# Dhia-naouali/dinov3-jax

Hardware: NVIDIA H100
Metric: global_crops_per_sec (higher is better)
Workload: dtype bf16

## Files before the change

dinov3-jax_b200/csrc/gemm_tc.cu:

```cuda
#include <cstdlib>
#include <cstring>
#include "ptx.cuh"
#include "d3_internal.h"

namespace d3 {

constexpr int BM = 128;
constexpr int BK = 64;
constexpr int GEMM_THREADS = 384;

constexpr int EPI_RUNTIME = -1;
constexpr int EPI_FLAGS = EP_BIAS | EP_GELU | EP_STORE_PRE | EP_MUL_DGELU | EP_GAMMA | EP_RESID | EP_OUT_F32 | EP_ACCUM |
                          EP_SLABS | EP_GELU_ERF;

template <int EF>
constexpr bool kStaged = EF != EPI_RUNTIME && (EF & (EP_SLABS | EP_ACCUM)) == 0;

template <int EF>
__device__ __forceinline__ bool epi_has(const GemmEpilogue& ep, int f) {
  return EF == EPI_RUNTIME ? (ep.flags & f) != 0 : (EF & f) != 0;
}

__device__ __forceinline__ float gelu_grad_epi(float u) {
  const float u2 = __fmul_rn(u, u);
  const float t = tanh_approx(__fmul_rn(u, fmaf(0.0356774081363001f, u2, 0.7978845608028654f)));
  const float dz = fmaf(0.1070322244089003f, u2, 0.7978845608028654f);
  return fmaf(__fmul_rn(__fmul_rn(0.5f, u), fmaf(-t, t, 1.0f)), dz, __fmul_rn(0.5f, __fadd_rn(1.0f, t)));
}

__device__ __forceinline__ float gelu_erf_epi(float u) {
  return __fmul_rn(__fmul_rn(0.5f, u), __fadd_rn(1.0f, erff(__fmul_rn(u, 0.70710678118654752f))));
}

template <int EF>
__device__ __forceinline__ float epi_value(const GemmEpilogue& ep, float acc, float bias, float u, float gamma,
                                           float resid, float old, float& pre) {
  float v = __fmul_rn(acc, ep.alpha);
  if (epi_has<EF>(ep, EP_BIAS)) v = __fadd_rn(v, bias);
  pre = v;
  if (epi_has<EF>(ep, EP_GELU)) v = gelu_tanh_fast(v);
  if (epi_has<EF>(ep, EP_GELU_ERF)) v = gelu_erf_epi(v);
  if (epi_has<EF>(ep, EP_MUL_DGELU)) v = __fmul_rn(v, gelu_grad_epi(u));
  if (epi_has<EF>(ep, EP_GAMMA)) v = __fmul_rn(v, gamma);
  if (epi_has<EF>(ep, EP_RESID)) v = __fadd_rn(v, resid);
  if (epi_has<EF>(ep, EP_ACCUM)) v = __fadd_rn(v, old);
  return v;
}

__device__ __forceinline__ float2 ld_pair(const float* p, bool vec, bool two) {
  if (vec) return *reinterpret_cast<const float2*>(p);
  return make_float2(p[0], two ? p[1] : 0.f);
}
__device__ __forceinline__ float2 ld_pair(const __nv_bfloat16* p, bool vec, bool two) {
  if (vec) return unpack_bf16(*reinterpret_cast<const uint32_t*>(p));
  return make_float2(__bfloat162float(p[0]), two ? __bfloat162float(p[1]) : 0.f);
}
__device__ __forceinline__ void st_pair(float* p, float a, float b, bool vec, bool two) {
  if (vec) {
    *reinterpret_cast<float2*>(p) = make_float2(a, b);
  } else {
    p[0] = a;
    if (two) p[1] = b;
  }
}
__device__ __forceinline__ void st_pair(__nv_bfloat16* p, float a, float b, bool vec, bool two) {
  if (vec) {
    *reinterpret_cast<uint32_t*>(p) = pack_bf16(a, b);
  } else {
    p[0] = __float2bfloat16(a);
    if (two) p[1] = __float2bfloat16(b);
  }
}

template <int BN>
__device__ __forceinline__ void epilogue_tile_runtime(const GemmEpilogue& ep, float (&acc)[2][BN / 2], int m0, int n0,
                                                      int M, int N, size_t slab_row0, int r_in, int c_in) {
  float* const out_f = reinterpret_cast<float*>(ep.out);
  __nv_bfloat16* const out_h = reinterpret_cast<__nv_bfloat16*>(ep.out);
  const bool aligned = (ep.flags & EP_SLOW) == 0;
#pragma unroll
  for (int mh = 0; mh < 2; ++mh)
#pragma unroll
    for (int h = 0; h < 2; ++h) {
      const size_t row = (size_t)(m0 + mh * 64 + r_in + 8 * h);
      if (row >= (size_t)M) continue;
      const size_t orow = slab_row0 + row;
#pragma unroll
      for (int i = 0; i < BN / 8; ++i) {
        const int n = n0 + 8 * i + c_in;
        if (n >= N) break;
        const bool two = n + 1 < N, vec = aligned && two;
        float2 b{}, u{}, g{}, x{}, o{};
        if (epi_has<EPI_RUNTIME>(ep, EP_BIAS)) b = ld_pair(ep.bias + n, vec, two);
        if (epi_has<EPI_RUNTIME>(ep, EP_MUL_DGELU)) u = ld_pair(ep.aux_in + row * ep.ld_aux + n, vec, two);
        if (epi_has<EPI_RUNTIME>(ep, EP_GAMMA)) g = ld_pair(ep.gamma + n, vec, two);
        if (epi_has<EPI_RUNTIME>(ep, EP_RESID)) x = ld_pair(ep.resid + row * ep.ld_resid + n, vec, two);
        if (epi_has<EPI_RUNTIME>(ep, EP_ACCUM)) o = ld_pair(out_f + orow * ep.ld_out + n, vec, two);
        float p0, p1;
        const float v0 = epi_value<EPI_RUNTIME>(ep, acc[mh][4 * i + 2 * h], b.x, u.x, g.x, x.x, o.x, p0);
        const float v1 = epi_value<EPI_RUNTIME>(ep, acc[mh][4 * i + 2 * h + 1], b.y, u.y, g.y, x.y, o.y, p1);
        if (epi_has<EPI_RUNTIME>(ep, EP_SCATTER)) {
          const unsigned long long g_idx = (unsigned long long)ep.sc_off + orow * ep.ld_out + n;
          const unsigned long long shard = (unsigned long long)ep.sc_shard;
          const unsigned r = (unsigned)(g_idx / shard);
          float* const dst = ep.sc_peer[r] + (g_idx - r * shard);
          if (!two) atomicAdd(dst, v0);
          else atomicAdd(reinterpret_cast<float2*>(dst), make_float2(v0, v1));
          continue;
        }
        if (epi_has<EPI_RUNTIME>(ep, EP_STORE_PRE)) st_pair(ep.aux_out + row * ep.ld_aux + n, p0, p1, vec, two);
        if (epi_has<EPI_RUNTIME>(ep, EP_OUT_F32)) st_pair(out_f + orow * ep.ld_out + n, v0, v1, vec, two);
        else st_pair(out_h + orow * ep.ld_out + n, v0, v1, vec, two);
      }
    }
}

constexpr int STG_BOX = 64 * 128;
constexpr int STG_BYTES = 3 * STG_BOX;
__device__ __forceinline__ uint32_t sw128(int r, int byte) {
  return r * 128 + ((((byte >> 4) ^ r) & 7) << 4) + (byte & 15);
}

template <int MH, int BN, int EF>
__device__ __forceinline__ void epilogue_tile(const GemmEpilogue& ep, const CUtensorMap* tm_out,
                                              const CUtensorMap* tm_pre, float (&acc)[MH][BN / 2], const float* s_bias,
                                              const float* s_gamma, uint8_t* stg, int& seq, int bar, int t, int m0,
                                              int n0, int M, int N, size_t slab_row0, int r_in, int c_in) {
  constexpr bool STAGED = kStaged<EF>;
  constexpr bool F32 = (EF & EP_OUT_F32) != 0;
  constexpr int OUT_BOXES = F32 ? 2 : 1;
  constexpr int CHUNK = (OUT_BOXES + ((EF & EP_STORE_PRE) ? 1 : 0)) * STG_BOX;
  constexpr int NBUF = STG_BYTES / CHUNK;
  static_assert(NBUF >= 1, "a chunk must fit the staging area");
  float* const out_f = reinterpret_cast<float*>(ep.out);
  __nv_bfloat16* const out_h = reinterpret_cast<__nv_bfloat16*>(ep.out);
#pragma unroll
  for (int mh = 0; mh < MH; ++mh)
#pragma unroll
    for (int cb = 0; cb < BN / 64; ++cb) {
      const int row0 = m0 + mh * 64, col0 = n0 + cb * 64;
      if (row0 >= M || col0 >= N) continue;
      float2 xr[2][8], xo[2][8];
      uint32_t xu[2][8];
#pragma unroll
      for (int h = 0; h < 2; ++h) {
        const size_t row = (size_t)row0 + r_in + 8 * h;
#pragma unroll
        for (int i = 0; i < 8; ++i) {
          const int n = col0 + 8 * i + c_in;
          if (row < (size_t)M && n < N) {
            if (epi_has<EF>(ep, EP_RESID))
              xr[h][i] = *reinterpret_cast<const float2*>(ep.resid + row * ep.ld_resid + n);
            if (epi_has<EF>(ep, EP_MUL_DGELU))
              xu[h][i] = *reinterpret_cast<const uint32_t*>(ep.aux_in + row * ep.ld_aux + n);
            if (epi_has<EF>(ep, EP_ACCUM))
              xo[h][i] = *reinterpret_cast<const float2*>(out_f + (slab_row0 + row) * ep.ld_out + n);
          }
        }
      }
      uint8_t* const buf = stg + (seq % NBUF) * CHUNK;
      if constexpr (STAGED) {
        if (t == 0) tma_store_wait_read<NBUF - 1>();
        named_bar_sync(bar, 128);
      }
#pragma unroll
      for (int h = 0; h < 2; ++h) {
        const int r = r_in + 8 * h;
        const size_t row = (size_t)row0 + r;
#pragma unroll
        for (int i = 0; i < 8; ++i) {
          const int cl = cb * 64 + 8 * i + c_in;
          const int n = n0 + cl;
          const float2 b = epi_has<EF>(ep, EP_BIAS) ? *reinterpret_cast<const float2*>(s_bias + cl) : float2{};
          const float2 g = epi_has<EF>(ep, EP_GAMMA) ? *reinterpret_cast<const float2*>(s_gamma + cl) : float2{};
          const float2 u = epi_has<EF>(ep, EP_MUL_DGELU) ? unpack_bf16(xu[h][i]) : float2{};
          float p0, p1;
          const float v0 = epi_value<EF>(ep, acc[mh][4 * (cl >> 3) + 2 * h], b.x, u.x, g.x, xr[h][i].x, xo[h][i].x, p0);
          const float v1 = epi_value<EF>(ep, acc[mh][4 * (cl >> 3) + 2 * h + 1], b.y, u.y, g.y, xr[h][i].y, xo[h][i].y,
                                         p1);
          if constexpr (STAGED) {
            if (epi_has<EF>(ep, EP_STORE_PRE))
              *reinterpret_cast<uint32_t*>(buf + OUT_BOXES * STG_BOX + sw128(r, 16 * i + 2 * c_in)) = pack_bf16(p0, p1);
            if constexpr (F32) {
              *reinterpret_cast<float2*>(buf + (i >> 2) * STG_BOX + sw128(r, 32 * (i & 3) + 4 * c_in)) =
                  make_float2(v0, v1);
            } else {
              *reinterpret_cast<uint32_t*>(buf + sw128(r, 16 * i + 2 * c_in)) = pack_bf16(v0, v1);
            }
          } else if (row < (size_t)M && n < N) {
            if (epi_has<EF>(ep, EP_STORE_PRE)) st_pair(ep.aux_out + row * ep.ld_aux + n, p0, p1, true, true);
            if constexpr (F32) st_pair(out_f + (slab_row0 + row) * ep.ld_out + n, v0, v1, true, true);
            else st_pair(out_h + (slab_row0 + row) * ep.ld_out + n, v0, v1, true, true);
          }
        }
      }
      if constexpr (STAGED) {
        fence_proxy_async_smem();
        named_bar_sync(bar, 128);
        if (t == 0) {
          tma_store_2d(tm_out, buf, col0, row0);
          if (F32 && col0 + 32 < N) tma_store_2d(tm_out, buf + STG_BOX, col0 + 32, row0);
          if constexpr ((EF & EP_STORE_PRE) != 0) tma_store_2d(tm_pre, buf + OUT_BOXES * STG_BOX, col0, row0);
          tma_store_commit();
        }
        ++seq;
      }
    }
}

template <int BN, bool STAGED>
struct Cfg {
  static constexpr bool WIDE = BN == 256;
  static constexpr int STAGES = (BN == 256 ? 4 : BN == 128 ? 6 : 8) - (STAGED ? 1 : 0);
  static constexpr int A_BYTES = BM * BK * 2;
  static constexpr int B_BYTES = BN * BK * 2;
  static constexpr int STAGE_BYTES = A_BYTES + B_BYTES;
  static constexpr int BAR_BYTES = 256;
  static constexpr int VEC_BYTES = (WIDE ? 1 : 2) * 2 * BN * 4;
  static constexpr int VEC_END = STAGES * STAGE_BYTES + BAR_BYTES + VEC_BYTES;
  static constexpr int STG_OFF = (VEC_END + 1023) / 1024 * 1024;
  static constexpr int SMEM_BYTES = (STAGED ? STG_OFF + 2 * STG_BYTES : VEC_END) + 1024;
  static_assert(SMEM_BYTES <= 227 * 1024, "over the opt-in shared-memory limit");
};

struct WorkRange { int m0, n0, kb0, kb1, sp; };
template <int BN>
__device__ __forceinline__ WorkRange work_item(int w, int rank, int num_n, int num_tiles, int num_k, int splits) {
  const int tile = w % num_tiles, sp = w / num_tiles;
  const int per = (num_k + splits - 1) / splits;
  WorkRange r;
  if constexpr (BN == 256) {
    r.n0 = (tile % num_n) * BN;
    r.m0 = (2 * (tile / num_n) + rank) * BM;
  } else {
    r.n0 = (2 * (tile % num_n) + rank) * BN;
    r.m0 = (tile / num_n) * BM;
  }
  r.kb0 = sp * per;
  r.kb1 = min(num_k, r.kb0 + per);
  r.sp = sp;
  return r;
}

template <int MH, int BN, int A_MN, int B_MN>
__device__ __forceinline__ void mma_kblock(float (&acc)[MH][BN / 2], uint32_t sa, uint32_t sb, bool first) {
  const uint64_t bd = B_MN ? gmma_desc_sw128(sb, 8192, 1024) : gmma_desc_sw128(sb, 16, 1024);
  constexpr uint64_t a_adv = A_MN ? (2048 >> 4) : (32 >> 4);
  constexpr uint64_t b_adv = B_MN ? (2048 >> 4) : (32 >> 4);
#pragma unroll
  for (int k = 0; k < BK / 16; ++k) {
    const uint32_t sc = (first && k == 0) ? 0u : 1u;
#pragma unroll
    for (int mh = 0; mh < MH; ++mh) {
      const uint64_t ad = A_MN ? gmma_desc_sw128(sa + mh * 8192, 8192, 1024) : gmma_desc_sw128(sa + mh * 8192, 16, 1024);
      if constexpr (BN == 256) wgmma_m64n256k16_ss<A_MN, B_MN>(acc[mh], ad + k * a_adv, bd + k * b_adv, sc);
      else if constexpr (BN == 128) wgmma_m64n128k16_ss<A_MN, B_MN>(acc[mh], ad + k * a_adv, bd + k * b_adv, sc);
      else wgmma_m64n64k16_ss<A_MN, B_MN>(acc[mh], ad + k * a_adv, bd + k * b_adv, sc);
    }
  }
}

template <int MH, int BN>
__device__ __forceinline__ void mma_khalf_e4m3(float (&acc)[MH][BN / 2], uint32_t sa, uint32_t sb, int h) {
  static_assert(BN == 64, "the e4m3 GEMM runs 128 x 64 tiles");
  const uint64_t bd = gmma_desc_sw128(sb, 16, 1024);
#pragma unroll
  for (int k = 0; k < 2; ++k) {
#pragma unroll
    for (int mh = 0; mh < MH; ++mh) {
      const uint64_t ad = gmma_desc_sw128(sa + mh * 8192, 16, 1024);
      wgmma_m64n64k32_e4m3(acc[mh], ad + (2 * h + k) * (32 >> 4), bd + (2 * h + k) * (32 >> 4), k == 0 ? 0u : 1u);
    }
  }
}

template <int MH, int BN>
__device__ __forceinline__ void add_acc(float (&acc)[MH][BN / 2], const float (&part)[MH][BN / 2]) {
#pragma unroll
  for (int mh = 0; mh < MH; ++mh)
#pragma unroll
    for (int i = 0; i < BN / 2; ++i) acc[mh][i] = __fadd_rn(acc[mh][i], part[mh][i]);
}

template <int BN, int A_MN, int B_MN, int EF, bool E4M3 = false>
__global__ void __launch_bounds__(GEMM_THREADS, 1)
gemm_kernel(const __grid_constant__ CUtensorMap tmA, const __grid_constant__ CUtensorMap tmB,
            const __grid_constant__ CUtensorMap tmO, const __grid_constant__ CUtensorMap tmP, const GemmEpilogue ep,
            int M, int N, int K, int splits, const float* scale_a, const float* scale_b) {
  static_assert(!E4M3 || (BN == 64 && !A_MN && !B_MN), "e4m3: 128 x 64 tiles, both operands K-major");
  constexpr int KB = E4M3 ? 128 : BK;
  constexpr bool staged = kStaged<EF>;
  using C = Cfg<BN, staged>;
  constexpr bool WIDE = C::WIDE;
  constexpr int MH = WIDE ? 1 : 2;
  static_assert(!WIDE || EF != EPI_RUNTIME, "run-time flags run on the 128-wide tile");
  static_assert(2 * C::STAGES * 8 <= C::BAR_BYTES, "mbarriers overflow their slot");
  extern __shared__ uint8_t smem_raw[];
  uint8_t* smem = reinterpret_cast<uint8_t*>((reinterpret_cast<uintptr_t>(smem_raw) + 1023) & ~uintptr_t(1023));
  uint64_t* full_bar = reinterpret_cast<uint64_t*>(smem + C::STAGES * C::STAGE_BYTES);
  uint64_t* empty_bar = full_bar + C::STAGES;
  float* vecs = reinterpret_cast<float*>(smem + C::STAGES * C::STAGE_BYTES + C::BAR_BYTES);

  const int wg = threadIdx.x >> 7;
  const int rank = blockIdx.x & 1;
  const int cluster = blockIdx.x >> 1, num_clusters = gridDim.x >> 1;
  if (threadIdx.x == 0) {
    tma_prefetch_desc(&tmA);
    tma_prefetch_desc(&tmB);
    if constexpr (staged) {
      tma_prefetch_desc(&tmO);
      if constexpr ((EF & EP_STORE_PRE) != 0) tma_prefetch_desc(&tmP);
    }
    for (int s = 0; s < C::STAGES; ++s) { mbar_init(&full_bar[s], 1); mbar_init(&empty_bar[s], WIDE ? 4 : 2); }
    fence_mbar_init();
  }
  cluster_sync();

  const int num_m = (M + BM - 1) / BM;
  const int num_n = WIDE ? (N + BN - 1) / BN : ((N + BN - 1) / BN + 1) / 2;
  const int num_k = (K + KB - 1) / KB;
  const int num_tiles = (WIDE ? (num_m + 1) / 2 : num_m) * num_n;
  const int num_work = num_tiles * splits;

  if (wg == 0) {
    setmaxnreg_dec<40>();
    if (threadIdx.x < 32 && elect_one()) {
      int stage = 0;
      uint32_t phase = 0;
      for (int w = cluster; w < num_work; w += num_clusters) {
        const WorkRange wr = work_item<BN>(w, rank, num_n, num_tiles, num_k, splits);
        for (int kb = wr.kb0; kb < wr.kb1; ++kb) {
          mbar_wait(&empty_bar[stage], phase ^ 1);
          uint8_t* sa = smem + stage * C::STAGE_BYTES;
          uint8_t* sb = sa + C::A_BYTES;
          mbar_expect_tx(&full_bar[stage], C::STAGE_BYTES);
          if constexpr (WIDE) {
#pragma unroll
            for (int i = 0; i < 2; ++i) {
              if (A_MN) tma_load_2d(&tmA, &full_bar[stage], sa + i * 8192, wr.m0 + i * 64, kb * KB);
              else tma_load_2d(&tmA, &full_bar[stage], sa + i * 8192, kb * KB, wr.m0 + i * 64);
            }
            if (B_MN) {
#pragma unroll
              for (int i = 2 * rank; i < 2 * rank + 2; ++i)
                tma_load_2d_multicast(&tmB, &full_bar[stage], sb + i * 8192, wr.n0 + i * 64, kb * KB, 0b11);
            } else {
              tma_load_2d_multicast(&tmB, &full_bar[stage], sb + rank * 16384, kb * KB, wr.n0 + rank * 128, 0b11);
            }
          } else {
            if (A_MN) {
              tma_load_2d_multicast(&tmA, &full_bar[stage], sa + rank * 8192, wr.m0 + rank * 64, kb * KB, 0b11);
            } else {
              tma_load_2d_multicast(&tmA, &full_bar[stage], sa + rank * 8192, kb * KB, wr.m0 + rank * 64, 0b11);
            }
            if (B_MN) {
#pragma unroll
              for (int i = 0; i < BN / 64; ++i) tma_load_2d(&tmB, &full_bar[stage], sb + i * 8192, wr.n0 + i * 64, kb * KB);
            } else {
              tma_load_2d(&tmB, &full_bar[stage], sb, kb * KB, wr.n0);
            }
          }
          if (++stage == C::STAGES) { stage = 0; phase ^= 1; }
        }
      }
    }
  } else {
    setmaxnreg_inc<232>();
    const int cw = wg - 1;
    const int t = threadIdx.x & 127;
    const int r_in = 16 * (t >> 5) + ((t & 31) >> 2);
    const int c_in = 2 * (t & 3);
    float* const s_bias = vecs + (WIDE ? 0 : cw * 2 * BN);
    float* const s_gamma = s_bias + BN;
    constexpr bool stage_vecs = EF != EPI_RUNTIME && (EF & (EP_BIAS | EP_GAMMA)) != 0;
    constexpr int VEC_THREADS = WIDE ? 256 : 128;
    const int vt = WIDE ? threadIdx.x - 128 : t;
    uint8_t* const stg = smem + C::STG_OFF + cw * STG_BYTES;
    const uint32_t peer_empty = mapa_shared(smem_u32(empty_bar), rank ^ 1);
    int stg_seq = 0;
    int stage = 0;
    uint32_t phase = 0;
    int j = 0;
    for (int w = cluster; w < num_work; w += num_clusters, ++j) {
      const WorkRange wr = work_item<BN>(w, rank, num_n, num_tiles, num_k, splits);
      const int nkb = wr.kb1 > wr.kb0 ? wr.kb1 - wr.kb0 : 0;
      if (!WIDE && (j & 1) != cw) {
        stage += nkb;
        phase ^= (stage / C::STAGES) & 1;
        stage %= C::STAGES;
        continue;
      }
      if constexpr (stage_vecs) {
        named_bar_sync(3 + cw * !WIDE, VEC_THREADS);
        if (vt < BN && wr.n0 + vt < N) {
          if constexpr ((EF & EP_BIAS) != 0) cp_async_4(s_bias + vt, ep.bias + wr.n0 + vt);
          if constexpr ((EF & EP_GAMMA) != 0) cp_async_4(s_gamma + vt, ep.gamma + wr.n0 + vt);
        }
      }
      if (!WIDE && j > 0) named_bar_sync(1 + cw, 256);
      float acc[MH][BN / 2];
#pragma unroll
      for (int mh = 0; mh < MH; ++mh)
#pragma unroll
        for (int i = 0; i < BN / 2; ++i) acc[mh][i] = 0.f;
      if constexpr (E4M3) {
        float part[MH][BN / 2];
        for (int kb = wr.kb0; kb < wr.kb1; ++kb) {
          mbar_wait(&full_bar[stage], phase);
          const uint32_t sa = smem_u32(smem + stage * C::STAGE_BYTES);
#pragma unroll
          for (int h = 0; h < 2; ++h) {
#pragma unroll
            for (int mh = 0; mh < MH; ++mh) fence_regs(part[mh]);
            wgmma_fence();
            mma_khalf_e4m3<MH, BN>(part, sa, sa + C::A_BYTES, h);
            wgmma_commit();
            wgmma_wait<0>();
#pragma unroll
            for (int mh = 0; mh < MH; ++mh) fence_regs(part[mh]);
            if (h == 1 && t == 0) { mbar_arrive(&empty_bar[stage]); mbar_arrive_cluster(peer_empty + 8 * stage); }
            add_acc<MH, BN>(acc, part);
          }
          if (++stage == C::STAGES) { stage = 0; phase ^= 1; }
        }
        if (!WIDE && w + num_clusters < num_work) named_bar_arrive(1 + (cw ^ 1), 256);
#pragma unroll
        for (int mh = 0; mh < MH; ++mh)
#pragma unroll
          for (int h = 0; h < 2; ++h) {
            const int row = wr.m0 + mh * 64 + r_in + 8 * h;
            const float s_row = row < M ? scale_a[row] : 0.f;
#pragma unroll
            for (int i = 0; i < BN / 8; ++i) {
              const int n = wr.n0 + 8 * i + c_in;
              const float s0 = n < N ? scale_b[n] : 0.f, s1 = n + 1 < N ? scale_b[n + 1] : 0.f;
              acc[mh][4 * i + 2 * h] = __fmul_rn(__fmul_rn(acc[mh][4 * i + 2 * h], s_row), s0);
              acc[mh][4 * i + 2 * h + 1] = __fmul_rn(__fmul_rn(acc[mh][4 * i + 2 * h + 1], s_row), s1);
            }
          }
      } else {
        int prev = -1;
        for (int kb = wr.kb0; kb < wr.kb1; ++kb) {
          mbar_wait(&full_bar[stage], phase);
          const uint32_t sa = smem_u32(smem + stage * C::STAGE_BYTES);
#pragma unroll
          for (int mh = 0; mh < MH; ++mh) fence_regs(acc[mh]);
          wgmma_fence();
          mma_kblock<MH, BN, A_MN, B_MN>(acc, sa + (WIDE ? cw * 8192 : 0), sa + C::A_BYTES, kb == wr.kb0);
          wgmma_commit();
#pragma unroll
          for (int mh = 0; mh < MH; ++mh) fence_regs(acc[mh]);
          if (prev >= 0) {
            wgmma_wait<1>();
            if (t == 0) { mbar_arrive(&empty_bar[prev]); mbar_arrive_cluster(peer_empty + 8 * prev); }
          }
          prev = stage;
          if (++stage == C::STAGES) { stage = 0; phase ^= 1; }
        }
        if (!WIDE && w + num_clusters < num_work) named_bar_arrive(1 + (cw ^ 1), 256);
        wgmma_wait<0>();
#pragma unroll
        for (int mh = 0; mh < MH; ++mh) fence_regs(acc[mh]);
        if (prev >= 0 && t == 0) { mbar_arrive(&empty_bar[prev]); mbar_arrive_cluster(peer_empty + 8 * prev); }
      }
      if constexpr (stage_vecs) {
        cp_async_wait_all();
        named_bar_sync(3 + cw * !WIDE, VEC_THREADS);
      }
      if (nkb <= 0) continue;
      const size_t slab_row0 = epi_has<EF>(ep, EP_SLABS) ? (size_t)wr.sp * M : 0;
      if constexpr (EF == EPI_RUNTIME) {
        epilogue_tile_runtime<BN>(ep, acc, wr.m0, wr.n0, M, N, slab_row0, r_in, c_in);
      } else {
        epilogue_tile<MH, BN, EF>(ep, &tmO, &tmP, acc, s_bias, s_gamma, stg, stg_seq, 5 + cw, t,
                                  wr.m0 + (WIDE ? cw * 64 : 0), wr.n0, M, N, slab_row0, r_in, c_in);
      }
    }
    if (staged && t == 0) tma_store_wait_all();
  }
  cluster_sync();
}

static int make_operand_map(CUtensorMap* map, const void* ptr, int mn, int k, int ld, int is_mn_major, int box_mn) {
  cuuint64_t dims[2], strides[1];
  cuuint32_t box[2], estr[2] = {1, 1};
  if (is_mn_major) {
    dims[0] = (cuuint64_t)mn; dims[1] = (cuuint64_t)k; box[0] = 64; box[1] = 64;
  } else {
    dims[0] = (cuuint64_t)k; dims[1] = (cuuint64_t)mn; box[0] = 64; box[1] = (cuuint32_t)box_mn;
  }
  strides[0] = (cuuint64_t)ld * 2;
  return encode_tensor_map_2d_bf16(map, ptr, dims, strides, box, estr);
}

template <int BN, int A_MN, int B_MN, int EF, bool E4M3 = false>
static int launch(const CUtensorMap& ta, const CUtensorMap& tb, const GemmEpilogue& ep, int M, int N, int K,
                  int splits, cudaStream_t stream, const float* scale_a = nullptr, const float* scale_b = nullptr) {
  using C = Cfg<BN, kStaged<EF>>;
  auto kern = gemm_kernel<BN, A_MN, B_MN, EF, E4M3>;
  cudaLaunchAttribute attr{};
  attr.id = cudaLaunchAttributeClusterDimension;
  attr.val.clusterDim.x = 2;
  attr.val.clusterDim.y = 1;
  attr.val.clusterDim.z = 1;
  cudaLaunchConfig_t cfg{};
  cfg.blockDim = dim3(GEMM_THREADS);
  cfg.dynamicSmemBytes = C::SMEM_BYTES;
  cfg.stream = stream;
  cfg.attrs = &attr;
  cfg.numAttrs = 1;
  static int max_clusters = 0;
  if (max_clusters == 0) {
    cudaError_t e = cudaFuncSetAttribute(kern, cudaFuncAttributeMaxDynamicSharedMemorySize, C::SMEM_BYTES);
    if (e != cudaSuccess) return set_error(D3_ERR_CUDA, cudaGetErrorString(e));
    cfg.gridDim = dim3(2 * sm_count());
    e = cudaOccupancyMaxActiveClusters(&max_clusters, kern, &cfg);
    if (e != cudaSuccess) return set_error(D3_ERR_CUDA, cudaGetErrorString(e));
    if (max_clusters < 1) return set_error(D3_ERR_CUDA, "gemm: no 2-CTA cluster fits on the device");
  }
  CUtensorMap to{}, tp{};
  if constexpr (kStaged<EF>) {
    const int elt = (EF & EP_OUT_F32) ? 4 : 2;
    int rc = encode_tensor_map_2d(&to, ep.out, elt, N, M, (cuuint64_t)ep.ld_out * elt, 128 / elt, 64, 128);
    if (rc) return rc;
    if constexpr ((EF & EP_STORE_PRE) != 0) {
      rc = encode_tensor_map_2d(&tp, ep.aux_out, 2, N, M, (cuuint64_t)ep.ld_aux * 2, 64, 64, 128);
      if (rc) return rc;
    }
  }
  const int num_m = (M + BM - 1) / BM, num_n = (N + BN - 1) / BN;
  const int work = (BN == 256 ? (num_m + 1) / 2 * num_n : num_m * ((num_n + 1) / 2)) * splits;
  cfg.gridDim = dim3(2 * (work < max_clusters ? work : max_clusters));
  cudaError_t e = cudaLaunchKernelEx(&cfg, kern, ta, tb, to, tp, ep, M, N, K, splits, scale_a, scale_b);
  if (e == cudaSuccess) e = cudaPeekAtLastError();
  if (e != cudaSuccess) return set_error(D3_ERR_CUDA, cudaGetErrorString(e));
  count_launch();
  return D3_OK;
}

template <int BN>
static int dispatch(int a_mn, int b_mn, const CUtensorMap& ta, const CUtensorMap& tb, const GemmEpilogue& ep, int M,
                    int N, int K, int splits, cudaStream_t s) {
  if (!(ep.flags & (EP_SLOW | EP_SCATTER)) && N % 2 == 0) {
    const int f = ep.flags & EPI_FLAGS;
#define D3_EPI(A, B, F) \
    if (a_mn == A && b_mn == B && f == (F)) return launch<BN, A, B, (F)>(ta, tb, ep, M, N, K, splits, s);
    D3_EPI(0, 1, 0)
    D3_EPI(0, 1, EP_BIAS)
    D3_EPI(0, 1, EP_BIAS | EP_OUT_F32)
    D3_EPI(0, 1, EP_BIAS | EP_GELU)
    D3_EPI(0, 1, EP_BIAS | EP_GELU | EP_STORE_PRE)
    D3_EPI(0, 1, EP_BIAS | EP_GAMMA | EP_RESID | EP_OUT_F32)
    D3_EPI(0, 1, EP_BIAS | EP_STORE_PRE | EP_GAMMA | EP_RESID | EP_OUT_F32)
    D3_EPI(0, 1, EP_BIAS | EP_GELU | EP_GAMMA | EP_RESID | EP_OUT_F32)
    D3_EPI(0, 1, EP_BIAS | EP_GELU | EP_STORE_PRE | EP_GAMMA | EP_RESID | EP_OUT_F32)
    D3_EPI(0, 1, EP_OUT_F32)
    D3_EPI(0, 1, EP_BIAS | EP_GELU_ERF)
    D3_EPI(0, 0, 0)
    D3_EPI(0, 0, EP_MUL_DGELU)
    D3_EPI(0, 0, EP_OUT_F32)
    D3_EPI(1, 1, EP_OUT_F32 | EP_SLABS)
    D3_EPI(1, 1, EP_OUT_F32 | EP_ACCUM)
#undef D3_EPI
  }
  if constexpr (BN == 256) {
    return dispatch<128>(a_mn, b_mn, ta, tb, ep, M, N, K, splits, s);
  } else {
    if (!a_mn && !b_mn) return launch<BN, 0, 0, EPI_RUNTIME>(ta, tb, ep, M, N, K, splits, s);
    if (!a_mn && b_mn) return launch<BN, 0, 1, EPI_RUNTIME>(ta, tb, ep, M, N, K, splits, s);
    if (a_mn && !b_mn) return launch<BN, 1, 0, EPI_RUNTIME>(ta, tb, ep, M, N, K, splits, s);
    return launch<BN, 1, 1, EPI_RUNTIME>(ta, tb, ep, M, N, K, splits, s);
  }
}

int gemm_bf16(const void* A, int lda, int a_mn, const void* B, int ldb, int b_mn, int M, int N, int K,
              GemmEpilogue ep, int tile_n, int split_k, cudaStream_t stream) {
  if (M <= 0 || N <= 0 || K <= 0) return set_error(D3_ERR_ARG, "gemm: empty problem");
  if ((lda % 8) || (ldb % 8) || (reinterpret_cast<uintptr_t>(A) & 15) || (reinterpret_cast<uintptr_t>(B) & 15))
    return set_error(D3_ERR_ARG, "gemm: operands must be 16-byte aligned with ld % 8 == 0");
  const int sms = sm_count();
  const int num_k = (K + BK - 1) / BK;
  int bn = tile_n >= 256 ? 256 : tile_n;
  if (tile_n == 0) {
    const int cand[2] = {128, 64};
    long best = -1;
    for (int i = 0; i < 2; ++i) {
      const long tiles = (long)((M + BM - 1) / BM) * ((N + cand[i] - 1) / cand[i]);
      const long waves = (tiles + sms - 1) / sms;
      const long cost = waves * (cand[i] + 24);
      if (best < 0 || cost < best) { best = cost; bn = cand[i]; }
    }
  }
  const bool plain_f32 = (ep.flags & EP_OUT_F32) && !(ep.flags & (EP_BIAS | EP_GELU | EP_STORE_PRE | EP_MUL_DGELU |
                                                                  EP_GAMMA | EP_RESID | EP_GELU_ERF));
  int splits = 1;
  if (split_k >= 1) {
    splits = split_k;
  } else if (plain_f32 && (ep.flags & EP_ACCUM)) {
    const int unit_n = bn < 128 ? bn : 128;
    const long units = (long)((M + BM - 1) / BM) * ((N + unit_n - 1) / unit_n);
    if (units <= sms && num_k >= 16) {
      splits = units * 2 <= sms ? (int)(sms / units) : 1;
      if (splits < (num_k + 63) / 64) splits = (num_k + 63) / 64;
      if (splits > num_k / 4) splits = num_k / 4;
      if (splits < 1) splits = 1;
    }
  }
  if (tile_n == 0 && a_mn && b_mn) bn = 256;
  if (ep.flags & EP_SCATTER) {
    if (!plain_f32) return set_error(D3_ERR_ARG, "gemm: SCATTER needs a plain fp32 output");
    if (ep.sc_world < 1 || ep.sc_world > 8 || ep.sc_shard <= 0 || (ep.sc_shard % 4) || (ep.sc_off % 4) || (ep.ld_out % 4))
      return set_error(D3_ERR_ARG, "gemm: SCATTER needs 1..8 ranks and 4-element aligned shard / offset / ld_out");
    if ((unsigned long long)ep.sc_off + (unsigned long long)(M - 1) * ep.ld_out + N > (unsigned long long)ep.sc_shard * ep.sc_world)
      return set_error(D3_ERR_ARG, "gemm: SCATTER output exceeds the sharded range");
  }
  if (splits > 1) {
    if (!plain_f32) return set_error(D3_ERR_ARG, "gemm: split-K needs a plain fp32 output");
    if (!(ep.flags & EP_ACCUM)) return set_error(D3_ERR_ARG, "gemm: split-K accumulates into out (set ACCUM, zero it first)");
    if (splits > num_k) splits = num_k;
  }
  if (ep.flags & EP_SCATTER) ep.flags &= ~EP_ACCUM;
  const int out_elt = (ep.flags & EP_OUT_F32) ? 4 : 2;
  bool aligned = ((uintptr_t)ep.out % 16 == 0) && ((ep.ld_out * out_elt) % 16 == 0);
  if (ep.flags & EP_BIAS) aligned = aligned && ((uintptr_t)ep.bias % 16 == 0);
  if (ep.flags & EP_GAMMA) aligned = aligned && ((uintptr_t)ep.gamma % 16 == 0);
  if (ep.flags & EP_RESID) aligned = aligned && ((uintptr_t)ep.resid % 16 == 0) && (ep.ld_resid % 4 == 0);
  if (ep.flags & EP_STORE_PRE) aligned = aligned && ((uintptr_t)ep.aux_out % 16 == 0) && (ep.ld_aux % 8 == 0);
  if (ep.flags & EP_MUL_DGELU) aligned = aligned && ((uintptr_t)ep.aux_in % 16 == 0) && (ep.ld_aux % 8 == 0);
  if (!aligned) ep.flags |= EP_SLOW;

  CUtensorMap ta, tb;
  int rc = make_operand_map(&ta, A, M, K, lda, a_mn, 64);
  if (rc) return rc;
  rc = make_operand_map(&tb, B, N, K, ldb, b_mn, bn < 128 ? bn : 128);
  if (rc) return rc;
  float* ws = nullptr;
  GemmEpilogue out_ep = ep;
  if (splits > 1 && !(ep.flags & EP_SCATTER)) {
    ws = slab_workspace((size_t)splits * M * N, stream);
    if (!ws) return D3_ERR_CUDA;
    ep.out = ws;
    ep.ld_out = N;
    ep.flags = (ep.flags & ~(EP_ACCUM | EP_SLOW)) | EP_SLABS | (N % 4 ? EP_SLOW : 0);
  }
  switch (bn) {
    case 256: rc = dispatch<256>(a_mn, b_mn, ta, tb, ep, M, N, K, splits, stream); break;
    case 128: rc = dispatch<128>(a_mn, b_mn, ta, tb, ep, M, N, K, splits, stream); break;
    case 64: rc = dispatch<64>(a_mn, b_mn, ta, tb, ep, M, N, K, splits, stream); break;
    default: rc = set_error(D3_ERR_ARG, "gemm: bad tile N");
  }
  if (ws) {
    if (!rc) rc = slab_combine(ws, splits, (long long)M * N, M, N, reinterpret_cast<float*>(out_ep.out), out_ep.ld_out, stream);
    slab_release(ws, stream);
  }
  return rc;
}

static int dispatch_e4m3(const CUtensorMap& ta, const CUtensorMap& tb, const GemmEpilogue& ep, int M, int N, int K,
                         const float* sa, const float* sb, cudaStream_t s) {
  if (!(ep.flags & EP_SLOW) && N % 2 == 0) {
    const int f = ep.flags & EPI_FLAGS;
#define D3_EPI(F) \
    if (f == (F)) return launch<64, 0, 0, (F), true>(ta, tb, ep, M, N, K, 1, s, sa, sb);
    D3_EPI(0)
    D3_EPI(EP_BIAS)
    D3_EPI(EP_BIAS | EP_GELU)
    D3_EPI(EP_BIAS | EP_GELU | EP_STORE_PRE)
    D3_EPI(EP_BIAS | EP_GAMMA | EP_RESID | EP_OUT_F32)
    D3_EPI(EP_BIAS | EP_STORE_PRE | EP_GAMMA | EP_RESID | EP_OUT_F32)
    D3_EPI(EP_BIAS | EP_GELU | EP_GAMMA | EP_RESID | EP_OUT_F32)
    D3_EPI(EP_BIAS | EP_GELU | EP_STORE_PRE | EP_GAMMA | EP_RESID | EP_OUT_F32)
    D3_EPI(EP_MUL_DGELU)
    D3_EPI(EP_OUT_F32)
    D3_EPI(EP_OUT_F32 | EP_ACCUM)
#undef D3_EPI
  }
  return launch<64, 0, 0, EPI_RUNTIME, true>(ta, tb, ep, M, N, K, 1, s, sa, sb);
}

int gemm_e4m3(const void* A, int lda, const float* sa, const void* B, int ldb, const float* sb, int M, int N, int K,
              GemmEpilogue ep, cudaStream_t stream) {
  if (M <= 0 || N <= 0 || K <= 0) return set_error(D3_ERR_ARG, "gemm_e4m3: empty problem");
  if (K % 16) return set_error(D3_ERR_ARG, "gemm_e4m3: K must be a multiple of 16");
  if ((lda % 16) || (ldb % 16) || (reinterpret_cast<uintptr_t>(A) & 15) || (reinterpret_cast<uintptr_t>(B) & 15))
    return set_error(D3_ERR_ARG, "gemm_e4m3: operands must be 16-byte aligned with ld % 16 == 0");
  if (ep.flags & (EP_SCATTER | EP_GELU_ERF)) return set_error(D3_ERR_ARG, "gemm_e4m3: SCATTER / GELU_ERF not supported");
  const int out_elt = (ep.flags & EP_OUT_F32) ? 4 : 2;
  bool aligned = ((uintptr_t)ep.out % 16 == 0) && ((ep.ld_out * out_elt) % 16 == 0);
  if (ep.flags & EP_BIAS) aligned = aligned && ((uintptr_t)ep.bias % 16 == 0);
  if (ep.flags & EP_GAMMA) aligned = aligned && ((uintptr_t)ep.gamma % 16 == 0);
  if (ep.flags & EP_RESID) aligned = aligned && ((uintptr_t)ep.resid % 16 == 0) && (ep.ld_resid % 4 == 0);
  if (ep.flags & EP_STORE_PRE) aligned = aligned && ((uintptr_t)ep.aux_out % 16 == 0) && (ep.ld_aux % 8 == 0);
  if (ep.flags & EP_MUL_DGELU) aligned = aligned && ((uintptr_t)ep.aux_in % 16 == 0) && (ep.ld_aux % 8 == 0);
  if (!aligned) ep.flags |= EP_SLOW;
  CUtensorMap ta, tb;
  int rc = encode_tensor_map_2d_u8(&ta, A, K, M, lda, 128, 64);
  if (rc) return rc;
  rc = encode_tensor_map_2d_u8(&tb, B, K, N, ldb, 128, 64);
  if (rc) return rc;
  return dispatch_e4m3(ta, tb, ep, M, N, K, sa, sb, stream);
}

}
```

Measured before the change: 553.0.

## Prefetch epilogue residual/aux inputs ahead of the mainloop and subsequent subtiles

Epilogue global loads for residual, dgelu aux and accumulate inputs are moved into a reusable EpiIn buffer. For staged epilogues, the first AH subtiles are preloaded before the MMA mainloop, and the next subtile is loaded while the current one is stored. This hides global load latency behind tensor-core work and TMA stores. In exchange it keeps the prefetched values live across the mainloop, which raises register pressure and risks spills. The prefetch depth is chosen per epilogue flag set to limit that cost.

After: 557.1, median of 6. Within noise of the previous version (+0.7%).

```diff
diff --git a/dinov3-jax_b200/csrc/gemm_tc.cu b/dinov3-jax_b200/csrc/gemm_tc.cu
--- a/dinov3-jax_b200/csrc/gemm_tc.cu
+++ b/dinov3-jax_b200/csrc/gemm_tc.cu
@@ -121,43 +121,74 @@
   return r * 128 + ((((byte >> 4) ^ r) & 7) << 4) + (byte & 15);
 }
 
+struct EpiIn {
+  float2 xr[2][8], xo[2][8];
+  uint32_t xu[2][8];
+};
+
+template <int EF>
+__device__ __forceinline__ void epi_load(const GemmEpilogue& ep, EpiIn& x, int row0, int col0, int M, int N,
+                                         size_t slab_row0, int r_in, int c_in) {
+  if (row0 >= M || col0 >= N) return;
+  const float* const out_f = reinterpret_cast<const float*>(ep.out);
+#pragma unroll
+  for (int h = 0; h < 2; ++h) {
+    const size_t row = (size_t)row0 + r_in + 8 * h;
+#pragma unroll
+    for (int i = 0; i < 8; ++i) {
+      const int n = col0 + 8 * i + c_in;
+      if (row < (size_t)M && n < N) {
+        if (epi_has<EF>(ep, EP_RESID)) x.xr[h][i] = *reinterpret_cast<const float2*>(ep.resid + row * ep.ld_resid + n);
+        if (epi_has<EF>(ep, EP_MUL_DGELU)) x.xu[h][i] = *reinterpret_cast<const uint32_t*>(ep.aux_in + row * ep.ld_aux + n);
+        if (epi_has<EF>(ep, EP_ACCUM))
+          x.xo[h][i] = *reinterpret_cast<const float2*>(out_f + (slab_row0 + row) * ep.ld_out + n);
+      }
+    }
+  }
+}
+
 template <int MH, int BN, int EF>
+constexpr int kAhead = !kStaged<EF> ? 1
+                       : (EF & EP_RESID) ? ((EF & EP_GELU) ? 1 : 2)
+                       : (EF & EP_MUL_DGELU) ? MH * BN / 64 : 1;
+
+template <int MH, int BN, int EF, int AH>
+__device__ __forceinline__ void epi_preload(const GemmEpilogue& ep, EpiIn (&x)[AH], int m0, int n0, int M, int N,
+                                            int r_in, int c_in) {
+  if constexpr (kStaged<EF>) {
+#pragma unroll
+    for (int c = 0; c < AH; ++c) epi_load<EF>(ep, x[c], m0 + (c / (BN / 64)) * 64, n0 + (c % (BN / 64)) * 64, M, N, 0, r_in, c_in);
+  }
+}
+
+template <int MH, int BN, int EF, int AH>
 __device__ __forceinline__ void epilogue_tile(const GemmEpilogue& ep, const CUtensorMap* tm_out,
-                                              const CUtensorMap* tm_pre, float (&acc)[MH][BN / 2], const float* s_bias,
-                                              const float* s_gamma, uint8_t* stg, int& seq, int bar, int t, int m0,
-                                              int n0, int M, int N, size_t slab_row0, int r_in, int c_in) {
+                                              const CUtensorMap* tm_pre, float (&acc)[MH][BN / 2], EpiIn (&xs)[AH],
+                                              const float* s_bias, const float* s_gamma, uint8_t* stg, int& seq,
+                                              int bar, int t, int m0, int n0, int M, int N, size_t slab_row0, int r_in,
+                                              int c_in) {
   constexpr bool STAGED = kStaged<EF>;
   constexpr bool F32 = (EF & EP_OUT_F32) != 0;
   constexpr int OUT_BOXES = F32 ? 2 : 1;
   constexpr int CHUNK = (OUT_BOXES + ((EF & EP_STORE_PRE) ? 1 : 0)) * STG_BOX;
   constexpr int NBUF = STG_BYTES / CHUNK;
+  constexpr int CB = BN / 64;
   static_assert(NBUF >= 1, "a chunk must fit the staging area");
   float* const out_f = reinterpret_cast<float*>(ep.out);
   __nv_bfloat16* const out_h = reinterpret_cast<__nv_bfloat16*>(ep.out);
 #pragma unroll
   for (int mh = 0; mh < MH; ++mh)
 #pragma unroll
-    for (int cb = 0; cb < BN / 64; ++cb) {
+    for (int cb = 0; cb < CB; ++cb) {
       const int row0 = m0 + mh * 64, col0 = n0 + cb * 64;
-      if (row0 >= M || col0 >= N) continue;
-      float2 xr[2][8], xo[2][8];
-      uint32_t xu[2][8];
-#pragma unroll
-      for (int h = 0; h < 2; ++h) {
-        const size_t row = (size_t)row0 + r_in + 8 * h;
-#pragma unroll
-        for (int i = 0; i < 8; ++i) {
-          const int n = col0 + 8 * i + c_in;
-          if (row < (size_t)M && n < N) {
-            if (epi_has<EF>(ep, EP_RESID))
-              xr[h][i] = *reinterpret_cast<const float2*>(ep.resid + row * ep.ld_resid + n);
-            if (epi_has<EF>(ep, EP_MUL_DGELU))
-              xu[h][i] = *reinterpret_cast<const uint32_t*>(ep.aux_in + row * ep.ld_aux + n);
-            if (epi_has<EF>(ep, EP_ACCUM))
-              xo[h][i] = *reinterpret_cast<const float2*>(out_f + (slab_row0 + row) * ep.ld_out + n);
-          }
-        }
-      }
+      const int c = mh * CB + cb, cn = c + AH;
+      EpiIn& x = xs[c % AH];
+      if (row0 >= M || col0 >= N) {
+        if constexpr (STAGED)
+          if (cn < MH * CB) epi_load<EF>(ep, x, m0 + (cn / CB) * 64, n0 + (cn % CB) * 64, M, N, 0, r_in, c_in);
+        continue;
+      }
+      if constexpr (!STAGED) epi_load<EF>(ep, x, row0, col0, M, N, slab_row0, r_in, c_in);
       uint8_t* const buf = stg + (seq % NBUF) * CHUNK;
       if constexpr (STAGED) {
         if (t == 0) tma_store_wait_read<NBUF - 1>();
@@ -173,11 +204,12 @@
           const int n = n0 + cl;
           const float2 b = epi_has<EF>(ep, EP_BIAS) ? *reinterpret_cast<const float2*>(s_bias + cl) : float2{};
           const float2 g = epi_has<EF>(ep, EP_GAMMA) ? *reinterpret_cast<const float2*>(s_gamma + cl) : float2{};
-          const float2 u = epi_has<EF>(ep, EP_MUL_DGELU) ? unpack_bf16(xu[h][i]) : float2{};
+          const float2 u = epi_has<EF>(ep, EP_MUL_DGELU) ? unpack_bf16(x.xu[h][i]) : float2{};
           float p0, p1;
-          const float v0 = epi_value<EF>(ep, acc[mh][4 * (cl >> 3) + 2 * h], b.x, u.x, g.x, xr[h][i].x, xo[h][i].x, p0);
-          const float v1 = epi_value<EF>(ep, acc[mh][4 * (cl >> 3) + 2 * h + 1], b.y, u.y, g.y, xr[h][i].y, xo[h][i].y,
-                                         p1);
+          const float v0 = epi_value<EF>(ep, acc[mh][4 * (cl >> 3) + 2 * h], b.x, u.x, g.x, x.xr[h][i].x, x.xo[h][i].x,
+                                         p0);
+          const float v1 = epi_value<EF>(ep, acc[mh][4 * (cl >> 3) + 2 * h + 1], b.y, u.y, g.y, x.xr[h][i].y,
+                                         x.xo[h][i].y, p1);
           if constexpr (STAGED) {
             if (epi_has<EF>(ep, EP_STORE_PRE))
               *reinterpret_cast<uint32_t*>(buf + OUT_BOXES * STG_BOX + sw128(r, 16 * i + 2 * c_in)) = pack_bf16(p0, p1);
@@ -195,6 +227,7 @@
         }
       }
       if constexpr (STAGED) {
+        if (cn < MH * CB) epi_load<EF>(ep, x, m0 + (cn / CB) * 64, n0 + (cn % CB) * 64, M, N, 0, r_in, c_in);
         fence_proxy_async_smem();
         named_bar_sync(bar, 128);
         if (t == 0) {
@@ -397,6 +430,9 @@
           if constexpr ((EF & EP_GAMMA) != 0) cp_async_4(s_gamma + vt, ep.gamma + wr.n0 + vt);
         }
       }
+      constexpr int AH = kAhead<MH, BN, EF>;
+      EpiIn xs[AH];
+      if constexpr (!E4M3) epi_preload<MH, BN, EF>(ep, xs, wr.m0 + (WIDE ? cw * 64 : 0), wr.n0, M, N, r_in, c_in);
       if (!WIDE && j > 0) named_bar_sync(1 + cw, 256);
       float acc[MH][BN / 2];
 #pragma unroll
@@ -424,6 +460,7 @@
           if (++stage == C::STAGES) { stage = 0; phase ^= 1; }
         }
         if (!WIDE && w + num_clusters < num_work) named_bar_arrive(1 + (cw ^ 1), 256);
+        epi_preload<MH, BN, EF>(ep, xs, wr.m0, wr.n0, M, N, r_in, c_in);
 #pragma unroll
         for (int mh = 0; mh < MH; ++mh)
 #pragma unroll
@@ -472,7 +509,7 @@
       if constexpr (EF == EPI_RUNTIME) {
         epilogue_tile_runtime<BN>(ep, acc, wr.m0, wr.n0, M, N, slab_row0, r_in, c_in);
       } else {
-        epilogue_tile<MH, BN, EF>(ep, &tmO, &tmP, acc, s_bias, s_gamma, stg, stg_seq, 5 + cw, t,
+        epilogue_tile<MH, BN, EF, AH>(ep, &tmO, &tmP, acc, xs, s_bias, s_gamma, stg, stg_seq, 5 + cw, t,
                                   wr.m0 + (WIDE ? cw * 64 : 0), wr.n0, M, N, slab_row0, r_in, c_in);
       }
     }
```
